# NVIDIA-Genomics-Research/GenomeWorks

Hardware: AMD Instinct MI355X
Metric: cudapoa consensus GCUPS, 1024-window short-read batch (static band 256, 32 reads <= 1024 bp) (higher is better)
Workload: dtype int16; 1 GPU; BASELINE configs[2]: cudapoa single-batch consensus, 1024 windows x 32 reads, backbone 960 bp, <=48 sub/24 ins/24 del, BatchConfig(1024,32,256,static_band), scores 8/-6/-8; windows_per_gpu=1024, cells_per_gpu=10990578176, parallelism=index-split x1

## Files before the change

genomeworks_amd/csrc/poa_forward_moves.h:

```cpp
#pragma once

#include "poa_forward_row_operands.h"

namespace gwhip
{

constexpr int kKindShift = 60;
constexpr uint32_t kMoveHoriz = 1;

__device__ __forceinline__ uint32_t pk_mad_u16_vsv(uint32_t a, uint32_t s, uint32_t c)
{
    uint32_t d;
    asm("v_pk_mad_u16 %0, %1, %2, %3" : "=v"(d) : "v"(a), "s"(s), "v"(c));
    return d;
}
__device__ __forceinline__ uint32_t pk_mad_u16_vvs(uint32_t a, uint32_t b, uint32_t s)
{
    uint32_t d;
    asm("v_pk_mad_u16 %0, %1, %2, %3" : "=v"(d) : "v"(a), "v"(b), "s"(s));
    return d;
}
__device__ __forceinline__ void gstore_nt_u64(void* p, uint32_t lo, uint32_t hi)
{
    u32x2 v;
    v.x = lo; v.y = hi;
    __builtin_nontemporal_store(v, reinterpret_cast<u32x2*>(p));
}
__device__ __forceinline__ void gstore_u16_lane0_below(const void* vptr, uint32_t v)
{
    asm volatile("s_mov_b64 exec, 1\n\tglobal_store_short %0, %1, off offset:-2\n\ts_mov_b64 exec, -1" ::"v"(vptr), "v"(v) : "memory");
}

template <int MAXD = kPkMaxDist, bool TBRULES = false>
__device__ __forceinline__ int32_t classify_kinds(RowInfo<true>* rowinfo, int32_t graph_count, int lane, const uint64_t* xpred, int32_t dbg = 0)
{
    int32_t first_moved = graph_count + 1;
    const bool demote_many = (dbg & (1 << 30)) != 0 && (dbg & (1 << 13)) == 0;
    for (int32_t r = 1 + lane; r <= graph_count; r += kWave)
    {
        RowInfo<true> ri  = rowinfo[r];
        const int32_t cnt = ri.cnt(), bs = ri.bs();
        uint64_t kind     = 4;
        const uint64_t xe  = (cnt > 3 && cnt <= 6 && xpred != nullptr) ? xpred[r & 255] : 0ull;
        const bool many_ok = cnt > 3 && cnt <= 6 && xpred_hit(xe, r, cnt) && !demote_many;
        if (cnt >= 1 && (cnt <= 3 || many_ok))
        {
            bool ok    = true;
            int32_t d0 = 0, pbs0 = 0;
            for (int32_t k = 0; k < cnt; k++)
            {
                const int32_t p   = k < 3 ? ri.pred(k) : xpred_row(xe, k);
                const int32_t d   = r - p;
                const RowInfo<true> pri = rowinfo[p];
                const int32_t pbs = pri.bs();
                ok                = ok && d >= 1 && d <= MAXD && (bs - pbs) <= kPkGuardCols && (bs == 0 || pbs > 0);
                if constexpr (TBRULES) ok = ok && !(pri.cnt() == 0 && pbs > 0);
                if (k == 0) { d0 = d; pbs0 = pbs; }
            }
            if (ok) kind = cnt > 1 ? 3 : ((d0 == 1 && pbs0 == bs) ? 0 : ((d0 == 1 && bs - pbs0 == kCellsPerLane) ? 1 : 2));
        }
        if ((dbg & 1024) && kind <= 1) kind = 2;
        if ((dbg & 32768) && kind == 1) kind = 2;
        if ((dbg & 512) && (kind == 2 || kind == 3)) kind = 4;
        if ((dbg & 2048) && kind <= 1) kind = 4;
        ri.w       = (ri.w & ~(7ull << kKindShift)) | (kind << kKindShift);
        rowinfo[r] = ri;
        if (bs > 0) first_moved = min(first_moved, r);
    }
    for (int off = 32; off > 0; off >>= 1) first_moved = min(first_moved, __shfl_xor(first_moved, off));
    return __builtin_amdgcn_readfirstlane(first_moved);
}

constexpr uint64_t kRowScoresInHbm = 1ull << 63;
template <typename IdT>
__device__ __forceinline__ void mark_score_rows(const GraphView<IdT>& g, RowInfo<true>* rowinfo, int32_t graph_count, int lane, bool all_rows)
{
    auto mark = [&](int32_t row) {
        __hip_atomic_fetch_or(reinterpret_cast<uint32_t*>(&rowinfo[row].w) + 1, 0x80000000u, __ATOMIC_RELAXED, __HIP_MEMORY_SCOPE_WORKGROUP);
    };
    for (int32_t r = 1 + lane; r <= graph_count; r += kWave)
    {
        const uint64_t w    = rowinfo[r].w;
        const uint32_t kind = (uint32_t)(w >> kKindShift) & 7u;
        const int32_t cnt   = (int32_t)((w >> 8) & 0x3fu);
        const bool reads_or_recomputes = kind >= 4u || cnt > 3;
        if (reads_or_recomputes || ((w >> 14) & 1u) != 0 || all_rows) mark(r);
        if (reads_or_recomputes)
        {
            const int32_t node_id = cnt > 3 ? (int32_t)g.sorted_poa[r - 1] : 0;
            for (int32_t k = 0; k < cnt; k++)
                mark(k < 3 ? (int32_t)((w >> (24 + 12 * k)) & 0xfffu) : (int32_t)g.node_id_to_pos[g.incoming_edges[(int64_t)node_id * kEdges + k]] + 1);
        }
    }
    wave_sync();
}
__device__ __forceinline__ bool row_recompute_safe(uint64_t w)
{
    return ((uint32_t)(w >> kKindShift) & 7u) >= 4u || ((w >> 8) & 0x3fu) > 3u || ((w >> 15) & 0x1ffu) == 0u;
}

template <typename IdT, int BW>
__device__ __forceinline__ void banded_forward_moves(const GraphView<IdT>& g, RowInfo<true>* rowinfo, int32_t graph_count,
                                                     const uint8_t* lds_read, int16_t* scores, uint8_t* moves, uint8_t* ring,
                                                     const uint64_t* xpred, int32_t max_column, int32_t gap_score,
                                                     int32_t mismatch_score, int32_t match_score, int32_t dbg,
                                                     uint64_t* prof_acc, bool store_all = true)
{
    const bool abl       = (dbg & (1 << 14)) != 0;
    const bool st_scores = !(abl && (dbg & (1 << 26))), st_moves = !(abl && (dbg & (1 << 27)));
    const bool ab_ring = !(abl && (dbg & (1 << 20))), ab_guard = !(abl && (dbg & (1 << 19))), ab_scan = !(abl && (dbg & (1 << 18))),
               ab_moves = !(abl && (dbg & (1 << 17))), ab_rows = !(abl && (dbg & (1 << 16)));
    const int32_t ksel = prof_acc ? ((dbg >> 28) & 7) - 1 : -1;
    const bool kfine   = (dbg & (1 << 13)) != 0;
    const bool kcount  = (dbg & (1 << 12)) != 0;
    uint64_t kacc      = 0;
    auto kselected = [&](uint32_t dk) -> bool { return ksel == (int32_t)((kfine || dk < kDkRingThree) ? dk : (uint32_t)kDkRingTwo); };
    const bool ksel_prev = kselected(kDkPrev), ksel_moved = kselected(kDkPrevMoved), ksel_one = kselected(kDkRingOne),
               ksel_two = kselected(kDkRingTwo), ksel_three = kselected(kDkRingThree), ksel_many = kselected(kDkRingMany),
               ksel_general = kselected(kDkGeneral);
    static_assert(kRowOpSlots == kPkSlots && kRowOpSlotBytes == kPkSlotBytes, "the row operands fold the ring's geometry in");
    static_assert(BW == 128 || BW == 256, "band widths of the packed pass");
    constexpr int32_t band_width = BW;
    constexpr int32_t stride     = band_width + kRightPad;
    constexpr int kBandLanes     = BW / kCellsPerLane;
    const int lane               = threadIdx.x & (kWave - 1);
    const bool band_lane         = lane < kBandLanes;
    const int32_t lane4 = lane * 4, lane8 = lane * 8;
    const int32_t min_score = Limits<int16_t>::min / 2;

    const int32_t first_moved = classify_kinds(rowinfo, graph_count, lane, xpred, dbg);
    wave_sync();
    mark_score_rows<IdT>(g, rowinfo, graph_count, lane, store_all);

    const uint32_t MIN2   = pin_vgpr(pk_dup(min_score));
    const uint32_t SENT2  = pin_vgpr(pk_dup(kPkSentinel));
    const uint32_t GAP2   = pin_vgpr(pk_dup(gap_score));
    const uint32_t MAT2   = pin_vgpr(pk_dup(match_score));
    const uint32_t DIF2   = pin_vgpr(pk_dup(mismatch_score - match_score));
    const uint32_t ONE2   = pin_vgpr(0x00010001u);
    const uint32_t THREE2 = pin_vgpr(0x00030003u);
    const uint32_t NEG1   = pin_vgpr(0xffffffffu);
    const uint32_t K01 = pk_make((lane4 + 0) * gap_score, (lane4 + 1) * gap_score);
    const uint32_t K23 = pk_make((lane4 + 2) * gap_score, (lane4 + 3) * gap_score);
    const uint32_t ring_base = lds_addr(ring);
    const uint32_t read_base = lds_addr(lds_read);
    const uint32_t guard_off  = lane < 16 ? (uint32_t)(2 * BW) : (lane == 16 ? (uint32_t)-136 : (uint32_t)(120 - 16 * lane));
    const bool is_lane16      = lane == 16;
    const bool is_lane63      = lane == kBandLanes - 1;
    const uint32_t move_keep  = lane == 0 ? 0xffffff00u : 0xffffffffu;
    const uint32_t GUARD_HI_MIN = pin_vgpr(is_lane16 ? (((uint32_t)kPkSentinel & 0xffffu) | ((uint32_t)min_score << 16)) : pk_dup(kPkSentinel));
    const uint32_t S0X_MIN      = (uint32_t)min_score << 16;

    uint32_t P01 = pk_make((lane4 + 1) * gap_score, (lane4 + 2) * gap_score);
    uint32_t P23 = pk_make((lane4 + 3) * gap_score, (lane4 + 4) * gap_score);
    int32_t prev_rel0 = 0;
    uint32_t rd4  = lds_load_u32(read_base + lane4);
    uint32_t rd4n = lds_load_u32(read_base + lane4 + 4);
    uint32_t a1   = (uint32_t)lane8;
    uint32_t ga   = (a1 + guard_off) & (kPkSlotBytes - 1);
    uint8_t* const score_base = reinterpret_cast<uint8_t*>(scores) + lane8 + 2 * (1 + kRelShift);
    uint8_t* const move_base  = moves + lane4 + (1 + kRelShift);

    if (BW == 256 || band_lane) lds_store_u64(ring_base + a1, P01, P23);
    lds_store_guard(ring_base + ga, SENT2, is_lane16 ? (((uint32_t)kPkSentinel & 0xffffu) | (0u << 16)) : SENT2);

    auto scan_row = [&](uint32_t s01, uint32_t s23, int32_t cu) {
        const uint32_t u01 = pk_sub(s01, K01), u23 = pk_sub(s23, K23);
        const uint32_t pm01 = pk_max(u01, (u01 << 16) | 0x8000u);
        const uint32_t pm23 = pk_max(u23, (u23 << 16) | 0x8000u);
        const int32_t m3    = (int32_t)pk_max(pm01, pm23) >> 16;
        const int32_t incl  = ab_scan ? wave_inclusive_max(m3) : m3;
        const int32_t excl  = max(wave_shr1(incl, cu), cu);
        const uint32_t ex2  = __builtin_amdgcn_perm((uint32_t)excl, (uint32_t)excl, 0x01000100u);
        const uint32_t m1b  = __builtin_amdgcn_perm(pm01, pm01, 0x03020302u);
        P01 = pk_add(pk_max(pm01, ex2), K01);
        P23 = pk_add(pk_max(pk_max(pm23, m1b), ex2), K23);
    };
    auto nz = [&](uint32_t a, uint32_t b) -> uint32_t { return pk_min_u16(pk_sub(a, b), ONE2); };
    auto costs = [&](uint32_t base4, uint32_t& c01, uint32_t& c23) {
        const uint32_t x   = rd4 ^ base4;
        const uint32_t x01 = __builtin_amdgcn_perm(0u, x, 0x0c010c00u);
        const uint32_t x23 = __builtin_amdgcn_perm(0u, x, 0x0c030c02u);
        c01 = pk_mad_u16(pk_min_u16(x01, ONE2), DIF2, MAT2);
        c23 = pk_mad_u16(pk_min_u16(x23, ONE2), DIF2, MAT2);
    };
    auto from_pred = [&](uint32_t s0x, uint32_t q01, uint32_t q23, uint32_t c01, uint32_t c23, uint32_t& D01, uint32_t& D23,
                         uint32_t& V01, uint32_t& V23) {
        D01 = pk_add(__builtin_amdgcn_alignbit(q01, s0x, 16), c01);
        D23 = pk_add(__builtin_amdgcn_alignbit(q23, q01, 16), c23);
        V01 = pk_add(q01, GAP2);
        V23 = pk_add(q23, GAP2);
    };
    auto store_row = [&](auto bs0_tag, int32_t r, int32_t rel0_val, uint32_t mv4, bool scores_to_hbm) {
        constexpr bool BS0 = decltype(bs0_tag)::value;
        const uint32_t sbase = ring_base + (((uint32_t)r & (kPkSlots - 1)) * kPkSlotBytes);
        if (BS0 || __builtin_expect(scores_to_hbm, 0))
        {
            uint8_t* score_ptr = score_base + (uint32_t)r * (uint32_t)(stride * 2);
            if (st_scores && (BW == 256 || band_lane)) gstore_nt_u64(score_ptr, P01, P23);
            if constexpr (BS0) gstore_u16_lane0_below(score_ptr, (uint32_t)rel0_val);
        }
        if (ab_ring && (BW == 256 || band_lane)) lds_store_u64(sbase + a1, P01, P23);
        if constexpr (BS0)
        {
            const uint32_t rel0pk = ((uint32_t)kPkSentinel & 0xffffu) | ((uint32_t)rel0_val << 16);
            if (ab_guard) lds_store_guard(sbase + ga, SENT2, is_lane16 ? rel0pk : SENT2);
            prev_rel0 = rel0_val;
        }
        else if (ab_guard)
            lds_store_guard(sbase + ga, SENT2, GUARD_HI_MIN);
        if (st_moves && (BW == 256 || band_lane)) *reinterpret_cast<uint32_t*>(move_base + (uint32_t)r * (uint32_t)stride) = mv4;
    };
    auto pack_moves = [&](uint32_t m01, uint32_t m23) -> uint32_t {
        return __builtin_amdgcn_perm(m23, m01, 0x06040200u) & move_keep;
    };

    auto general_row = [&](int32_t r, int32_t& prev_rel0_io) {
        const RowInfo<true> ri = uniform_row(rowinfo[r]);
        const int32_t bs       = ri.bs();
        const uint32_t base    = (uint32_t)ri.base();
        const int32_t prev_bs  = r > 1 ? uniform_row(rowinfo[r - 1]).bs() : 0;
        a1   = (uint32_t)(2 * bs + lane8) & (kPkSlotBytes - 1);
        ga   = (a1 + guard_off) & (kPkSlotBytes - 1);
        rd4  = lds_load_u32(read_base + bs + lane4);
        rd4n = lds_load_u32(read_base + bs + lane4 + 4);
        const int32_t pred_count = ri.cnt();
        const int32_t c          = bs + lane4;
        const int32_t cp0 = ((rd4 & 0xff) == base) ? match_score : mismatch_score;
        const int32_t cp1 = (((rd4 >> 8) & 0xff) == base) ? match_score : mismatch_score;
        const int32_t cp2 = (((rd4 >> 16) & 0xff) == base) ? match_score : mismatch_score;
        const int32_t cp3 = ((rd4 >> 24) == base) ? match_score : mismatch_score;
        const int32_t R0 = pk_lo(P01), R1 = pk_hi(P01), R2 = pk_lo(P23), R3 = pk_hi(P23);
        bool synced = false;
        auto from_regs = [&](int32_t& t0, int32_t& t1, int32_t& t2, int32_t& t3) {
            const int32_t q    = (bs - prev_bs) >> 2;
            const int32_t pend = min(prev_bs + band_width - kCellsPerLane, max_column);
            const int src      = lane + q;
            const int32_t from_left = __shfl(R3, src - 1);
            const int32_t S0        = (q == 0 && lane == 0) ? prev_rel0_io : from_left;
            const int32_t S1 = __shfl(R0, src), S2 = __shfl(R1, src), S3 = __shfl(R2, src), S4 = __shfl(R3, src);
            const bool valid = c <= pend;
            t0 = valid ? max(S0 + cp0, S1 + gap_score) : min_score;
            t1 = valid ? max(S1 + cp1, S2 + gap_score) : min_score;
            t2 = valid ? max(S2 + cp2, S3 + gap_score) : min_score;
            t3 = valid ? max(S3 + cp3, S4 + gap_score) : min_score;
        };
        auto from_hbm = [&](int32_t prow, int32_t& t0, int32_t& t1, int32_t& t2, int32_t& t3) {
            const int32_t pbs  = prow == 0 ? 0 : uniform_row(rowinfo[prow]).bs();
            const int32_t pend = min(pbs + band_width - kCellsPerLane, max_column);
            const bool valid   = !(c > pend || c < pbs);
            if (!synced) { wave_sync(); synced = true; }
            const int16_t* rowp = scores + (int64_t)prow * stride + (valid ? (c - pbs) : 0) + kRelShift;
            int32_t S0 = rowp[0];
            const Quad<int16_t> qd = *reinterpret_cast<const Quad<int16_t>*>(rowp + 1);
            const int32_t S1 = qd.v[0], S2 = qd.v[1], S3 = qd.v[2], S4 = qd.v[3];
            if (pbs > 0 && c == pbs) S0 = min_score;
            t0 = valid ? max(S0 + cp0, S1 + gap_score) : min_score;
            t1 = valid ? max(S1 + cp1, S2 + gap_score) : min_score;
            t2 = valid ? max(S2 + cp2, S3 + gap_score) : min_score;
            t3 = valid ? max(S3 + cp3, S4 + gap_score) : min_score;
        };
        auto rel0_of = [&](int32_t prow) -> int32_t {
            if (prow == r - 1) return prev_rel0_io;
            const int32_t pbs = prow == 0 ? 0 : uniform_row(rowinfo[prow]).bs();
            if (pbs > 0) return min_score;
            if (!synced) { wave_sync(); synced = true; }
            return wave_first((int32_t)scores[(int64_t)prow * stride + kRelShift]);
        };
        const int32_t node_id = (pred_count > 3) ? (int32_t)g.sorted_poa[r - 1] : 0;
        auto pred_row = [&](int32_t p) -> int32_t {
            if (pred_count == 0) return 0;
            if (p < 3) return ri.pred(p);
            return wave_first((int32_t)g.node_id_to_pos[g.incoming_edges[(int64_t)node_id * kEdges + p]] + 1);
        };
        int32_t fe = 0, rel0_val = min_score;
        if (pred_count == 0)
        {
            if (bs == 0) rel0_val = gap_score;
        }
        else
        {
            if (bs > kCellsPerLane && pred_count == 1)
                fe = min_score + gap_score;
            else
            {
                int32_t penalty = min_score;
                for (int32_t p = 0; p < pred_count; p++) penalty = max(penalty, rel0_of(pred_row(p)));
                fe = penalty + gap_score;
            }
            if (bs == 0) rel0_val = fe;
        }
        int32_t s0 = 0, s1 = 0, s2 = 0, s3 = 0;
        const int32_t np = max(pred_count, 1);
        for (int32_t p = 0; p < np; p++)
        {
            const int32_t prow = pred_row(p);
            int32_t t0, t1, t2, t3;
            if (prow == r - 1) from_regs(t0, t1, t2, t3);
            else from_hbm(prow, t0, t1, t2, t3);
            if (p == 0) { s0 = t0; s1 = t1; s2 = t2; s3 = t3; }
            else { s0 = max(s0, t0); s1 = max(s1, t1); s2 = max(s2, t2); s3 = max(s3, t3); }
        }
        scan_row(pk_make(s0, s1), pk_make(s2, s3), fe + gap_score);
        uint8_t* score_ptr = score_base + (uint32_t)r * (uint32_t)(stride * 2);
        const uint32_t sbase  = ring_base + (((uint32_t)r & (kPkSlots - 1)) * kPkSlotBytes);
        const uint32_t rel0pk = ((uint32_t)kPkSentinel & 0xffffu) | ((uint32_t)rel0_val << 16);
        if (BW == 256 || band_lane)
        {
            *reinterpret_cast<uint2*>(score_ptr) = make_uint2(P01, P23);
            lds_store_u64(sbase + a1, P01, P23);
        }
        lds_store_guard(sbase + ga, SENT2, is_lane16 ? rel0pk : SENT2);
        if (bs == 0) gstore_u16_lane0_below(score_ptr, (uint32_t)rel0_val);
        if (BW == 256 || band_lane) *reinterpret_cast<uint32_t*>(move_base + (uint32_t)r * (uint32_t)stride) = 0u;
        prev_rel0_io = rel0_val;
    };

    auto reg_row = [&](auto bs0_tag, auto moved_tag, int32_t r, uint32_t d0, uint32_t base4, bool scores_to_hbm) {
        constexpr bool BS0   = decltype(bs0_tag)::value;
        constexpr bool MOVED = decltype(moved_tag)::value;
        uint32_t s0x, q01, q23;
        if constexpr (!MOVED)
        {
            s0x = (uint32_t)wave_shr1((int32_t)P23, BS0 ? (int32_t)((uint32_t)prev_rel0 << 16) : (int32_t)S0X_MIN);
            q01 = P01; q23 = P23;
        }
        else
        {
            s0x  = P23;
            q01  = (uint32_t)wave_shl1((int32_t)P01, (int32_t)pk_dup(kPkSentinel));
            q23  = (uint32_t)wave_shl1((int32_t)P23, (int32_t)pk_dup(kPkSentinel));
            a1   = (a1 + 8) & (kPkSlotBytes - 1);
            ga   = (ga + 8) & (kPkSlotBytes - 1);
            rd4  = rd4n;
            rd4n = lds_load_u32((d0 >> kRowOpReadShift) + lane4 + 4);
        }
        int32_t cu = min_score + 2 * gap_score, rel0_val = min_score;
        if constexpr (BS0)
        {
            rel0_val = max(min_score, prev_rel0) + gap_score;
            cu       = rel0_val + gap_score;
        }
        uint32_t c01, c23, D01, D23, V01, V23;
        costs(base4, c01, c23);
        from_pred(s0x, q01, q23, c01, c23, D01, D23, V01, V23);
        uint32_t s01 = pk_max(D01, V01), s23 = pk_max(D23, V23);
        if constexpr (MOVED)
        {
            s01 = is_lane63 ? MIN2 : s01;
            s23 = is_lane63 ? MIN2 : s23;
        }
        scan_row(s01, s23, cu);
        const uint32_t m01 = pk_mad_u16(nz(P01, D01), pk_mad_u16(nz(P01, V01), NEG1, NEG1), THREE2);
        const uint32_t m23 = pk_mad_u16(nz(P23, D23), pk_mad_u16(nz(P23, V23), NEG1, NEG1), THREE2);
        uint32_t mv4 = ab_moves ? pack_moves(m01, m23) : 0u;
        if constexpr (MOVED) mv4 = is_lane63 ? 0u : mv4;
        store_row(bs0_tag, r, rel0_val, mv4, scores_to_hbm);
    };

    auto ring_row = [&](auto bs0_tag, auto np_tag, int32_t r, int32_t k, uint32_t d0, uint32_t base4, const RowOperands& OPv) {
        constexpr bool BS0 = decltype(bs0_tag)::value;
        constexpr int NP   = decltype(np_tag)::value;
        auto fetch = [&](uint32_t v) -> uint32_t { return (uint32_t)__builtin_amdgcn_readlane((int32_t)v, k); };
        const uint32_t b0 = fetch(OPv.slot0), bs2 = fetch(OPv.bs2), m0 = fetch(OPv.mv0), m1 = fetch(OPv.mv1);
        const uint32_t b1 = NP >= 2 ? fetch(OPv.slot1) : 0u, m2 = NP >= 2 ? fetch(OPv.mv2) : 0u;
        const uint32_t b2 = NP >= 3 ? fetch(OPv.slot2) : 0u, m3 = NP >= 3 ? fetch(OPv.mv3) : 0u;
        const uint32_t rdb = (d0 >> kRowOpReadShift) + (uint32_t)lane4;
        const bool scores_to_hbm = (d0 & kRowOpScoresToHbm) != 0;
        a1 = (bs2 + (uint32_t)lane8) & (kPkSlotBytes - 1);
        ga = (a1 + guard_off) & (kPkSlotBytes - 1);
        const uint32_t a0     = (a1 - 4) & (kPkSlotBytes - 1);
        const uint32_t sent16 = (uint32_t)kPkSentinel & 0xffffu;
        auto rel0_in = [&](uint32_t b) -> int32_t { return (int32_t)(int16_t)wave_first((int32_t)(lds_load_u32(b + kPkSlotBytes - 4) >> 16)); };
        if constexpr (NP == 1)
        {
            const uint32_t x0 = lds_load_u32(b0 + a0);
            const uint2 q0    = lds_load_u64(b0 + a1);
            rd4  = lds_load_u32(rdb);
            rd4n = lds_load_u32(rdb + 4);
            int32_t cu = min_score + 2 * gap_score, rel0_val = min_score;
            if constexpr (BS0)
            {
                rel0_val = max(min_score, rel0_in(b0)) + gap_score;
                cu       = rel0_val + gap_score;
            }
            uint32_t c01, c23, D01, D23, V01, V23;
            costs(base4, c01, c23);
            from_pred(x0, q0.x, q0.y, c01, c23, D01, D23, V01, V23);
            const bool outside = (q0.x & 0xffffu) == sent16;
            const uint32_t s01 = pk_max(D01, V01), s23 = pk_max(D23, V23);
            scan_row(outside ? MIN2 : s01, outside ? MIN2 : s23, cu);
            const uint32_t m01 = pk_mad_u16_vvs(nz(P01, D01), pk_mad_u16_vsv(nz(P01, V01), m1, NEG1), m0);
            const uint32_t m23 = pk_mad_u16_vvs(nz(P23, D23), pk_mad_u16_vsv(nz(P23, V23), m1, NEG1), m0);
            const uint32_t mv4 = outside ? 0u : pack_moves(m01, m23);
            store_row(bs0_tag, r, rel0_val, mv4, scores_to_hbm);
        }
        else
        {
            const uint32_t x0 = lds_load_u32(b0 + a0);
            const uint2 q0    = lds_load_u64(b0 + a1);
            const uint32_t x1 = lds_load_u32(b1 + a0);
            const uint2 q1    = lds_load_u64(b1 + a1);
            uint32_t x2 = 0;
            uint2 q2 = make_uint2(0, 0);
            if constexpr (NP > 2)
            {
                x2 = lds_load_u32(b2 + a0);
                q2 = lds_load_u64(b2 + a1);
            }
            rd4  = lds_load_u32(rdb);
            rd4n = lds_load_u32(rdb + 4);
            int32_t fe = min_score + gap_score;
            if constexpr (BS0)
            {
                int32_t pen = max(min_score, rel0_in(b0));
                pen = max(pen, rel0_in(b1));
                if constexpr (NP > 2) pen = max(pen, rel0_in(b2));
                fe = pen + gap_score;
            }
            uint32_t c01, c23;
            costs(base4, c01, c23);
            uint32_t D0a, D0b, V0a, V0b, D1a, D1b, V1a, V1b;
            from_pred(x0, q0.x, q0.y, c01, c23, D0a, D0b, V0a, V0b);
            from_pred(x1, q1.x, q1.y, c01, c23, D1a, D1b, V1a, V1b);
            const bool out0 = (q0.x & 0xffffu) == sent16, out1 = (q1.x & 0xffffu) == sent16;
            bool undecided  = out0 | out1;
            D0a = out0 ? MIN2 : D0a; D0b = out0 ? MIN2 : D0b; V0a = out0 ? MIN2 : V0a; V0b = out0 ? MIN2 : V0b;
            D1a = out1 ? MIN2 : D1a; D1b = out1 ? MIN2 : D1b; V1a = out1 ? MIN2 : V1a; V1b = out1 ? MIN2 : V1b;
            uint32_t bD01 = pk_max(D0a, D1a), bD23 = pk_max(D0b, D1b), bV01 = pk_max(V0a, V1a), bV23 = pk_max(V0b, V1b);
            const uint32_t E1v = pin_vgpr(m2);
            uint32_t A01, A23, B01, B23;
            if constexpr (NP > 2)
            {
                uint32_t D2a, D2b, V2a, V2b;
                from_pred(x2, q2.x, q2.y, c01, c23, D2a, D2b, V2a, V2b);
                const bool out2 = (q2.x & 0xffffu) == sent16;
                undecided       = undecided | out2;
                D2a = out2 ? MIN2 : D2a; D2b = out2 ? MIN2 : D2b; V2a = out2 ? MIN2 : V2a; V2b = out2 ? MIN2 : V2b;
                bD01 = pk_max(bD01, D2a); bD23 = pk_max(bD23, D2b); bV01 = pk_max(bV01, V2a); bV23 = pk_max(bV23, V2b);
                const uint32_t E2 = pin_vgpr(m3);
                A01 = pk_mad_u16_vvs(nz(bD01, D0a), pk_mad_u16(nz(bD01, D1a), E2, E1v), m0);
                A23 = pk_mad_u16_vvs(nz(bD23, D0b), pk_mad_u16(nz(bD23, D1b), E2, E1v), m0);
                B01 = pk_mad_u16_vvs(nz(bV01, V0a), pk_mad_u16(nz(bV01, V1a), E2, E1v), m1);
                B23 = pk_mad_u16_vvs(nz(bV23, V0b), pk_mad_u16(nz(bV23, V1b), E2, E1v), m1);
            }
            else
            {
                A01 = pk_mad_u16_vvs(nz(bD01, D0a), E1v, m0); A23 = pk_mad_u16_vvs(nz(bD23, D0b), E1v, m0);
                B01 = pk_mad_u16_vvs(nz(bV01, V0a), E1v, m1); B23 = pk_mad_u16_vvs(nz(bV23, V0b), E1v, m1);
            }
            if constexpr (NP > 3)
            {
                const uint64_t xe     = wave_first64(xpred[r & 255]);
                const int32_t cnt_all = (int32_t)((xe >> 13) & 63u);
                uint32_t xD01 = MIN2, xD23 = MIN2, xV01 = MIN2, xV23 = MIN2;
                int32_t pen_x = min_score;
                for (int32_t kk = 3; kk < cnt_all; kk++)
                {
                    const uint32_t bk = ring_base + (((uint32_t)xpred_row(xe, kk) & 7u) * kPkSlotBytes);
                    const uint32_t xk = lds_load_u32(bk + a0);
                    const uint2 qk    = lds_load_u64(bk + a1);
                    uint32_t Da, Db, Va, Vb;
                    from_pred(xk, qk.x, qk.y, c01, c23, Da, Db, Va, Vb);
                    const bool outk = (qk.x & 0xffffu) == sent16;
                    undecided       = undecided | outk;
                    xD01 = pk_max(xD01, outk ? MIN2 : Da); xD23 = pk_max(xD23, outk ? MIN2 : Db);
                    xV01 = pk_max(xV01, outk ? MIN2 : Va); xV23 = pk_max(xV23, outk ? MIN2 : Vb);
                    if constexpr (BS0) pen_x = max(pen_x, rel0_in(bk));
                }
                if constexpr (BS0) fe = max(fe - gap_score, pen_x) + gap_score;
                const uint32_t fD01 = pk_max(bD01, xD01), fD23 = pk_max(bD23, xD23), fV01 = pk_max(bV01, xV01), fV23 = pk_max(bV23, xV23);
                A01 = pk_mad_u16(nz(bD01, fD01), pk_sub(0u, A01), A01); A23 = pk_mad_u16(nz(bD23, fD23), pk_sub(0u, A23), A23);
                B01 = pk_mad_u16(nz(bV01, fV01), pk_sub(0u, B01), B01); B23 = pk_mad_u16(nz(bV23, fV23), pk_sub(0u, B23), B23);
                bD01 = fD01; bD23 = fD23; bV01 = fV01; bV23 = fV23;
            }
            const int32_t rel0_val = BS0 ? fe : min_score;
            scan_row(pk_max(bD01, bV01), pk_max(bD23, bV23), fe + gap_score);
            auto move_of = [&](uint32_t H, uint32_t bD, uint32_t bV, uint32_t A, uint32_t B) -> uint32_t {
                const uint32_t t1 = pk_mad_u16(nz(H, bV), pk_sub(ONE2, B), B);
                return pk_mad_u16(nz(H, bD), pk_sub(t1, A), A);
            };
            const uint32_t m01 = move_of(P01, bD01, bV01, A01, B01);
            const uint32_t m23 = move_of(P23, bD23, bV23, A23, B23);
            const uint32_t mv4 = undecided ? 0u : pack_moves(m01, m23);
            store_row(bs0_tag, r, rel0_val, mv4, scores_to_hbm);
        }
    };

    constexpr int32_t kBlockRows = kWave - 1;
    auto run_rows = [&](auto bs0_tag, int32_t r_from, int32_t r_to) {
        constexpr bool BS0 = decltype(bs0_tag)::value;
        const uint64_t kone = !kfine ? 1ull : (BS0 ? 1ull << 32 : 1ull << 48);
        int32_t r = r_from;
        while (r <= r_to)
        {
            const int32_t rr     = min(r + lane, graph_count);
            const RowOperands OPv = pack_row_operands(rowinfo[rr].w, (uint32_t)rr, lane < kBlockRows && r + lane <= r_to, ring_base, read_base);
            const int32_t r0 = r;
            int32_t k        = 0;
            uint32_t d0, base4;
            auto fetch = [&]() {
                d0    = (uint32_t)__builtin_amdgcn_readlane((int32_t)OPv.d0, k);
                base4 = (uint32_t)__builtin_amdgcn_readlane((int32_t)OPv.base4, k);
            };
            auto timed = [&](auto dk_tag, bool selected, auto&& body) {
                const uint64_t t = selected ? clock64() : 0;
                body();
                if (selected) kacc += kcount ? kone : clock64() - t;
                k++;
                asm volatile("; end of a row of kind %0" ::"n"(decltype(dk_tag)::value));
            };
            for (;;)
            {
                fetch();
                const uint64_t t_k0 = ksel_prev ? clock64() : 0;
                const int32_t k_k0  = k;
                while ((d0 & 7u) == kDkPrev)
                {
                    reg_row(bs0_tag, std::false_type{}, r0 + k, d0, base4, (d0 & kRowOpScoresToHbm) != 0);
                    k++;
                    fetch();
                }
                if (ksel_prev) kacc += kcount ? (uint64_t)(k - k_k0) * kone : clock64() - t_k0;
                if (d0 & kRowOpIsRingTwo)
                {
                    timed(std::integral_constant<uint32_t, kDkRingTwo>{}, ksel_two, [&]() { ring_row(bs0_tag, std::integral_constant<int, 2>{}, r0 + k, k, d0, base4, OPv); });
                    continue;
                }
                if (d0 & kRowOpIsRingOne)
                {
                    timed(std::integral_constant<uint32_t, kDkRingOne>{}, ksel_one, [&]() { ring_row(bs0_tag, std::integral_constant<int, 1>{}, r0 + k, k, d0, base4, OPv); });
                    continue;
                }
                if (d0 & kRowOpIsPrevMoved)
                {
                    timed(std::integral_constant<uint32_t, kDkPrevMoved>{}, ksel_moved, [&]() { reg_row(bs0_tag, std::true_type{}, r0 + k, d0, base4, (d0 & kRowOpScoresToHbm) != 0); });
                    continue;
                }
                if (d0 & kRowOpIsEnd) break;
                const uint32_t kind = d0 & 7u;
                if (kind == kDkRingThree)
                {
                    timed(std::integral_constant<uint32_t, kDkRingThree>{}, ksel_three, [&]() { ring_row(bs0_tag, std::integral_constant<int, 3>{}, r0 + k, k, d0, base4, OPv); });
                    continue;
                }
                if (kind == kDkRingMany)
                {
                    timed(std::integral_constant<uint32_t, kDkRingMany>{}, ksel_many, [&]() { ring_row(bs0_tag, std::integral_constant<int, 4>{}, r0 + k, k, d0, base4, OPv); });
                    continue;
                }
                timed(std::integral_constant<uint32_t, kDkGeneral>{}, ksel_general, [&]() {
                    general_row(r0 + k, prev_rel0);
                    if constexpr (!BS0) prev_rel0 = min_score;
                });
            }
            r = r0 + k;
        }
    };

    const int32_t bs0_end = min(first_moved - 1, graph_count);
    if (!ab_rows) return;
    run_rows(std::true_type{}, 1, bs0_end);
    run_rows(std::false_type{}, bs0_end + 1, graph_count);
    if (ksel >= 0 && lane == 0) *prof_acc += kacc;
}

}
```

genomeworks_amd/csrc/poa_forward_row_operands.h:

```cpp
#pragma once

#include <cstdint>

#if defined(__HIPCC__)
#define GWHIP_ROW_OPERANDS_FN __host__ __device__ inline
#else
#define GWHIP_ROW_OPERANDS_FN inline
#endif

namespace gwhip
{

constexpr uint32_t kDkPrev = 0, kDkPrevMoved = 1, kDkRingOne = 2, kDkRingTwo = 3, kDkGeneral = 4, kDkRingThree = 5, kDkRingMany = 6,
                   kDkEnd = 7;
constexpr uint32_t kRowOpSlots = 8, kRowOpSlotBytes = 1024;
constexpr uint32_t kRowOpScoresToHbm = 1u << 3;
constexpr uint32_t kRowOpIsRingTwo = 1u << 4, kRowOpIsRingOne = 1u << 5, kRowOpIsPrevMoved = 1u << 6, kRowOpIsEnd = 1u << 7;
constexpr int kRowOpReadShift      = 8;

struct RowOperands
{
    uint32_t d0;
    uint32_t base4;
    uint32_t slot0, slot1, slot2;
    uint32_t bs2;
    uint32_t mv0, mv1, mv2, mv3;
};

GWHIP_ROW_OPERANDS_FN uint32_t row_operand_dup16(int32_t v) { return ((uint32_t)v & 0xffffu) | ((uint32_t)v << 16); }

GWHIP_ROW_OPERANDS_FN uint32_t row_descriptor_kind(uint32_t kind, uint32_t cnt)
{
    if (kind == 3u) return cnt == 2u ? kDkRingTwo : (cnt == 3u ? kDkRingThree : kDkRingMany);
    return kind > 4u ? kDkGeneral : kind;
}

GWHIP_ROW_OPERANDS_FN RowOperands pack_row_operands(uint64_t w, uint32_t row, bool in_block, uint32_t ring_base, uint32_t read_base)
{
    const uint32_t kind = (uint32_t)(w >> 60) & 7u;
    const uint32_t cnt  = (uint32_t)(w >> 8) & 0x3fu;
    const uint32_t bs   = ((uint32_t)(w >> 15) & 0x1ffu) << 2;
    const uint32_t p0 = (uint32_t)(w >> 24) & 0xfffu, p1 = (uint32_t)(w >> 36) & 0xfffu, p2 = (uint32_t)(w >> 48) & 0xfffu;
    const int32_t dd0 = (int32_t)((row - p0) & 7u), dd1 = (int32_t)((row - p1) & 7u), dd2 = (int32_t)((row - p2) & 7u);
    const uint32_t dk = in_block ? row_descriptor_kind(kind, cnt) : kDkEnd;
    RowOperands o;
    const uint32_t kind_bits = dk == kDkRingTwo ? kRowOpIsRingTwo : (dk == kDkRingOne ? kRowOpIsRingOne : (dk == kDkPrevMoved ? kRowOpIsPrevMoved : (dk == kDkEnd ? kRowOpIsEnd : 0u)));
    o.d0    = dk | ((uint32_t)(w >> 63) << 3) | kind_bits | ((read_base + bs) << kRowOpReadShift);
    o.base4 = ((uint32_t)w & 0xffu) * 0x01010101u;
    o.slot0 = ring_base + (p0 & (kRowOpSlots - 1)) * kRowOpSlotBytes;
    o.slot1 = ring_base + (p1 & (kRowOpSlots - 1)) * kRowOpSlotBytes;
    o.slot2 = ring_base + (p2 & (kRowOpSlots - 1)) * kRowOpSlotBytes;
    o.bs2   = 2u * bs;
    const bool one = kind == kDkRingOne;
    o.mv0 = row_operand_dup16(2 * dd0 + 1);
    o.mv1 = row_operand_dup16(one ? 1 - 2 * dd0 : 2 * dd0);
    o.mv2 = row_operand_dup16(2 * (dd1 - dd0));
    o.mv3 = row_operand_dup16(2 * (dd2 - dd1));
    return o;
}

}
```

Measured before the change: 431.3 GCUPS.

## Fuse sibling rows sharing one predecessor into a paired DPP scan

Rows of kind 'prev' that are followed by a ring-one sibling with the same single predecessor and the same band start are marked as pair leaders. Both rows are then computed together from the shared predecessor row. Their two wave-wide prefix-max scans are interleaved through a hand-written DPP sequence to hide latency and share the diagonal and vertical operands. New inline-constant v_pk_mad forms produce the sibling's move encoding. This adds extra VGPR pressure and per-block readlane and marking work.

```diff
diff --git a/genomeworks_amd/csrc/poa_forward_moves.h b/genomeworks_amd/csrc/poa_forward_moves.h
--- a/genomeworks_amd/csrc/poa_forward_moves.h
+++ b/genomeworks_amd/csrc/poa_forward_moves.h
@@ -18,6 +18,20 @@
 {
     uint32_t d;
     asm("v_pk_mad_u16 %0, %1, %2, %3" : "=v"(d) : "v"(a), "v"(b), "s"(s));
+    return d;
+}
+template <int C> __device__ __forceinline__ uint32_t pk_mad_u16_vcv(uint32_t a, uint32_t c)
+{
+    static_assert(C >= -16 && C <= 64, "an inline constant");
+    uint32_t d;
+    asm("v_pk_mad_u16 %0, %1, %2, %3 op_sel_hi:[1,0,1]" : "=v"(d) : "v"(a), "n"(C), "v"(c));
+    return d;
+}
+template <int C> __device__ __forceinline__ uint32_t pk_mad_u16_vvc(uint32_t a, uint32_t b)
+{
+    static_assert(C >= -16 && C <= 64, "an inline constant");
+    uint32_t d;
+    asm("v_pk_mad_u16 %0, %1, %2, %3 op_sel_hi:[1,1,0]" : "=v"(d) : "v"(a), "v"(b), "n"(C));
     return d;
 }
 __device__ __forceinline__ void gstore_nt_u64(void* p, uint32_t lo, uint32_t hi)
@@ -118,6 +132,8 @@
     const bool ksel_prev = kselected(kDkPrev), ksel_moved = kselected(kDkPrevMoved), ksel_one = kselected(kDkRingOne),
                ksel_two = kselected(kDkRingTwo), ksel_three = kselected(kDkRingThree), ksel_many = kselected(kDkRingMany),
                ksel_general = kselected(kDkGeneral);
+    const bool ksel_pair = prof_acc != nullptr && (dbg & (1u << 31)) != 0 && kfine && ((dbg >> 28) & 7) == 0;
+    const bool pairing   = (dbg & (1u << 31)) == 0 || ksel_pair;
     static_assert(kRowOpSlots == kPkSlots && kRowOpSlotBytes == kPkSlotBytes, "the row operands fold the ring's geometry in");
     static_assert(BW == 128 || BW == 256, "band widths of the packed pass");
     constexpr int32_t band_width = BW;
@@ -164,7 +180,7 @@
     if (BW == 256 || band_lane) lds_store_u64(ring_base + a1, P01, P23);
     lds_store_guard(ring_base + ga, SENT2, is_lane16 ? (((uint32_t)kPkSentinel & 0xffffu) | (0u << 16)) : SENT2);
 
-    auto scan_row = [&](uint32_t s01, uint32_t s23, int32_t cu) {
+    auto scan_into = [&](uint32_t s01, uint32_t s23, int32_t cu, uint32_t& R01, uint32_t& R23) {
         const uint32_t u01 = pk_sub(s01, K01), u23 = pk_sub(s23, K23);
         const uint32_t pm01 = pk_max(u01, (u01 << 16) | 0x8000u);
         const uint32_t pm23 = pk_max(u23, (u23 << 16) | 0x8000u);
@@ -173,9 +189,42 @@
         const int32_t excl  = max(wave_shr1(incl, cu), cu);
         const uint32_t ex2  = __builtin_amdgcn_perm((uint32_t)excl, (uint32_t)excl, 0x01000100u);
         const uint32_t m1b  = __builtin_amdgcn_perm(pm01, pm01, 0x03020302u);
-        P01 = pk_add(pk_max(pm01, ex2), K01);
-        P23 = pk_add(pk_max(pk_max(pm23, m1b), ex2), K23);
-    };
+        R01 = pk_add(pk_max(pm01, ex2), K01);
+        R23 = pk_add(pk_max(pk_max(pm23, m1b), ex2), K23);
+    };
+    auto scan_two_into = [&](uint32_t sa01, uint32_t sa23, uint32_t sb01, uint32_t sb23, int32_t cu, uint32_t& A01, uint32_t& A23,
+                             uint32_t& B01, uint32_t& B23) {
+        const uint32_t ua01 = pk_sub(sa01, K01), ub01 = pk_sub(sb01, K01), ua23 = pk_sub(sa23, K23), ub23 = pk_sub(sb23, K23);
+        const uint32_t pa01 = pk_max(ua01, (ua01 << 16) | 0x8000u), pb01 = pk_max(ub01, (ub01 << 16) | 0x8000u);
+        const uint32_t pa23 = pk_max(ua23, (ua23 << 16) | 0x8000u), pb23 = pk_max(ub23, (ub23 << 16) | 0x8000u);
+        int32_t va = (int32_t)pk_max(pa01, pa23) >> 16, vb = (int32_t)pk_max(pb01, pb23) >> 16;
+        if (ab_scan)
+        {
+            constexpr int32_t ident = INT32_MIN;
+#define GW_DPP_MAX2(ctrl, rmask)                                                        \
+    {                                                                                   \
+        const int32_t ta = __builtin_amdgcn_update_dpp(ident, va, ctrl, rmask, 0xf, false); \
+        const int32_t tb = __builtin_amdgcn_update_dpp(ident, vb, ctrl, rmask, 0xf, false); \
+        va = max(va, ta);                                                               \
+        vb = max(vb, tb);                                                               \
+    }
+            GW_DPP_MAX2(0x111, 0xf);
+            GW_DPP_MAX2(0x112, 0xf);
+            GW_DPP_MAX2(0x114, 0xf);
+            GW_DPP_MAX2(0x118, 0xf);
+            GW_DPP_MAX2(0x142, 0xa);
+            GW_DPP_MAX2(0x143, 0xc);
+#undef GW_DPP_MAX2
+        }
+        const int32_t ea = max(wave_shr1(va, cu), cu), eb = max(wave_shr1(vb, cu), cu);
+        const uint32_t xa = __builtin_amdgcn_perm((uint32_t)ea, (uint32_t)ea, 0x01000100u), xb = __builtin_amdgcn_perm((uint32_t)eb, (uint32_t)eb, 0x01000100u);
+        const uint32_t ma = __builtin_amdgcn_perm(pa01, pa01, 0x03020302u), mb = __builtin_amdgcn_perm(pb01, pb01, 0x03020302u);
+        A01 = pk_add(pk_max(pa01, xa), K01);
+        B01 = pk_add(pk_max(pb01, xb), K01);
+        A23 = pk_add(pk_max(pk_max(pa23, ma), xa), K23);
+        B23 = pk_add(pk_max(pk_max(pb23, mb), xb), K23);
+    };
+    auto scan_row = [&](uint32_t s01, uint32_t s23, int32_t cu) { scan_into(s01, s23, cu, P01, P23); };
     auto nz = [&](uint32_t a, uint32_t b) -> uint32_t { return pk_min_u16(pk_sub(a, b), ONE2); };
     auto costs = [&](uint32_t base4, uint32_t& c01, uint32_t& c23) {
         const uint32_t x   = rd4 ^ base4;
@@ -191,16 +240,16 @@
         V01 = pk_add(q01, GAP2);
         V23 = pk_add(q23, GAP2);
     };
-    auto store_row = [&](auto bs0_tag, int32_t r, int32_t rel0_val, uint32_t mv4, bool scores_to_hbm) {
+    auto store_row_of = [&](auto bs0_tag, int32_t r, int32_t rel0_val, uint32_t mv4, bool scores_to_hbm, uint32_t R01, uint32_t R23) {
         constexpr bool BS0 = decltype(bs0_tag)::value;
         const uint32_t sbase = ring_base + (((uint32_t)r & (kPkSlots - 1)) * kPkSlotBytes);
         if (BS0 || __builtin_expect(scores_to_hbm, 0))
         {
             uint8_t* score_ptr = score_base + (uint32_t)r * (uint32_t)(stride * 2);
-            if (st_scores && (BW == 256 || band_lane)) gstore_nt_u64(score_ptr, P01, P23);
+            if (st_scores && (BW == 256 || band_lane)) gstore_nt_u64(score_ptr, R01, R23);
             if constexpr (BS0) gstore_u16_lane0_below(score_ptr, (uint32_t)rel0_val);
         }
-        if (ab_ring && (BW == 256 || band_lane)) lds_store_u64(sbase + a1, P01, P23);
+        if (ab_ring && (BW == 256 || band_lane)) lds_store_u64(sbase + a1, R01, R23);
         if constexpr (BS0)
         {
             const uint32_t rel0pk = ((uint32_t)kPkSentinel & 0xffffu) | ((uint32_t)rel0_val << 16);
@@ -210,6 +259,9 @@
         else if (ab_guard)
             lds_store_guard(sbase + ga, SENT2, GUARD_HI_MIN);
         if (st_moves && (BW == 256 || band_lane)) *reinterpret_cast<uint32_t*>(move_base + (uint32_t)r * (uint32_t)stride) = mv4;
+    };
+    auto store_row = [&](auto bs0_tag, int32_t r, int32_t rel0_val, uint32_t mv4, bool scores_to_hbm) {
+        store_row_of(bs0_tag, r, rel0_val, mv4, scores_to_hbm, P01, P23);
     };
     auto pack_moves = [&](uint32_t m01, uint32_t m23) -> uint32_t {
         return __builtin_amdgcn_perm(m23, m01, 0x06040200u) & move_keep;
@@ -487,6 +539,27 @@
         }
     };
 
+    auto pair_rows = [&](int32_t r, uint32_t d0, uint32_t base4, uint32_t d0f, uint32_t base4f) {
+        const uint32_t s0x = (uint32_t)wave_shr1((int32_t)P23, (int32_t)S0X_MIN);
+        const int32_t cu   = min_score + 2 * gap_score;
+        uint32_t cA01, cA23, cB01, cB23;
+        costs(base4, cA01, cA23);
+        costs(base4f, cB01, cB23);
+        const uint32_t g01 = __builtin_amdgcn_alignbit(P01, s0x, 16), g23 = __builtin_amdgcn_alignbit(P23, P01, 16);
+        const uint32_t V01 = pk_add(P01, GAP2), V23 = pk_add(P23, GAP2);
+        const uint32_t DA01 = pk_add(g01, cA01), DA23 = pk_add(g23, cA23), DB01 = pk_add(g01, cB01), DB23 = pk_add(g23, cB23);
+        uint32_t A01, A23, B01, B23;
+        scan_two_into(pk_max(DA01, V01), pk_max(DA23, V23), pk_max(DB01, V01), pk_max(DB23, V23), cu, A01, A23, B01, B23);
+        const uint32_t mA01 = pk_mad_u16(nz(A01, DA01), pk_mad_u16(nz(A01, V01), NEG1, NEG1), THREE2);
+        const uint32_t mB01 = pk_mad_u16_vvc<5>(nz(B01, DB01), pk_mad_u16_vcv<-3>(nz(B01, V01), NEG1));
+        const uint32_t mA23 = pk_mad_u16(nz(A23, DA23), pk_mad_u16(nz(A23, V23), NEG1, NEG1), THREE2);
+        const uint32_t mB23 = pk_mad_u16_vvc<5>(nz(B23, DB23), pk_mad_u16_vcv<-3>(nz(B23, V23), NEG1));
+        const uint32_t mvA = ab_moves ? pack_moves(mA01, mA23) : 0u, mvB = ab_moves ? pack_moves(mB01, mB23) : 0u;
+        store_row_of(std::false_type{}, r, min_score, mvA, (d0 & kRowOpScoresToHbm) != 0, A01, A23);
+        store_row_of(std::false_type{}, r + 1, min_score, mvB, (d0f & kRowOpScoresToHbm) != 0, B01, B23);
+        P01 = B01; P23 = B23;
+    };
+
     constexpr int32_t kBlockRows = kWave - 1;
     auto run_rows = [&](auto bs0_tag, int32_t r_from, int32_t r_to) {
         constexpr bool BS0 = decltype(bs0_tag)::value;
@@ -495,7 +568,14 @@
         while (r <= r_to)
         {
             const int32_t rr     = min(r + lane, graph_count);
-            const RowOperands OPv = pack_row_operands(rowinfo[rr].w, (uint32_t)rr, lane < kBlockRows && r + lane <= r_to, ring_base, read_base);
+            const uint64_t w_row = rowinfo[rr].w;
+            RowOperands OPv      = pack_row_operands(w_row, (uint32_t)rr, lane < kBlockRows && r + lane <= r_to, ring_base, read_base);
+            if constexpr (!BS0)
+                if (pairing)
+                {
+                    const uint64_t w_next = ((uint64_t)(uint32_t)wave_shl1((int32_t)(uint32_t)(w_row >> 32), 0) << 32) | (uint32_t)wave_shl1((int32_t)(uint32_t)w_row, 0);
+                    OPv.d0 = mark_pair_leader(OPv, w_row, w_next, lane, lane + 1 < kBlockRows && r + lane + 1 <= r_to, true);
+                }
             const int32_t r0 = r;
             int32_t k        = 0;
             uint32_t d0, base4;
@@ -532,6 +612,20 @@
                     timed(std::integral_constant<uint32_t, kDkRingOne>{}, ksel_one, [&]() { ring_row(bs0_tag, std::integral_constant<int, 1>{}, r0 + k, k, d0, base4, OPv); });
                     continue;
                 }
+                if constexpr (!BS0)
+                    if (d0 & kRowOpIsPairLeader)
+                    {
+                        const uint64_t t = ksel_pair ? clock64() : 0;
+                        const uint32_t d0f    = (uint32_t)__builtin_amdgcn_readlane((int32_t)OPv.d0, k + 1);
+                        const uint32_t base4f = (uint32_t)__builtin_amdgcn_readlane((int32_t)OPv.base4, k + 1);
+                        pair_rows(r0 + k, d0, base4, d0f, base4f);
+                        if (ksel_pair) kacc += kcount ? kone : clock64() - t;
+                        if (kcount && ksel_prev) kacc += kone;
+                        if (kcount && ksel_one) kacc += kone;
+                        k += 2;
+                        asm volatile("; end of a sibling pair");
+                        continue;
+                    }
                 if (d0 & kRowOpIsPrevMoved)
                 {
                     timed(std::integral_constant<uint32_t, kDkPrevMoved>{}, ksel_moved, [&]() { reg_row(bs0_tag, std::true_type{}, r0 + k, d0, base4, (d0 & kRowOpScoresToHbm) != 0); });
@@ -562,7 +656,7 @@
     if (!ab_rows) return;
     run_rows(std::true_type{}, 1, bs0_end);
     run_rows(std::false_type{}, bs0_end + 1, graph_count);
-    if (ksel >= 0 && lane == 0) *prof_acc += kacc;
-}
-
-}
+    if ((ksel >= 0 || ksel_pair) && lane == 0) *prof_acc += kacc;
+}
+
+}
diff --git a/genomeworks_amd/csrc/poa_forward_row_operands.h b/genomeworks_amd/csrc/poa_forward_row_operands.h
--- a/genomeworks_amd/csrc/poa_forward_row_operands.h
+++ b/genomeworks_amd/csrc/poa_forward_row_operands.h
@@ -17,6 +17,10 @@
 constexpr uint32_t kRowOpScoresToHbm = 1u << 3;
 constexpr uint32_t kRowOpIsRingTwo = 1u << 4, kRowOpIsRingOne = 1u << 5, kRowOpIsPrevMoved = 1u << 6, kRowOpIsEnd = 1u << 7;
 constexpr int kRowOpReadShift      = 8;
+constexpr uint32_t kRowOpIsPairLeader = 1u << 31;
+constexpr uint32_t kRowOpLdsLimit = 160u << 10, kRowOpBandStartLimit = 0x1ffu << 2;
+constexpr int kRowOpPairLastLane  = 61;
+static_assert(((kRowOpLdsLimit + kRowOpBandStartLimit) << kRowOpReadShift) < kRowOpIsPairLeader, "the read address leaves d0's top bit free");
 
 struct RowOperands
 {
@@ -59,4 +63,14 @@
     return o;
 }
 
+GWHIP_ROW_OPERANDS_FN uint32_t mark_pair_leader(const RowOperands& o, uint64_t w, uint64_t w_next, int lane, bool next_in_block, bool moved_phase)
+{
+    const uint32_t next_kind = (uint32_t)(w_next >> 60) & 7u, next_cnt = (uint32_t)(w_next >> 8) & 0x3fu;
+    const bool same_pred = (((uint32_t)(w_next >> 24) ^ (uint32_t)(w >> 24)) & 0xfffu) == 0u;
+    const bool same_band = (((uint32_t)(w_next >> 15) ^ (uint32_t)(w >> 15)) & 0x1ffu) == 0u;
+    const bool leader = moved_phase && lane <= kRowOpPairLastLane && next_in_block && (o.d0 & (7u | kRowOpIsPairLeader)) == kDkPrev &&
+                        next_kind == kDkRingOne && next_cnt == 1u && same_pred && same_band;
+    return leader ? (o.d0 | kDkGeneral | kRowOpIsPairLeader) : o.d0;
 }
+
+}
```

Result: no change. 435.2 GCUPS (median of 6 runs) (+0.9%).
